# philbull/FastBox

Measured on AMD Instinct MI355X. Metric: 512^3 box realisations/sec (gen + log-normal + P(k)), higher is better.
Workload: dtype f32

## Files before the change

fastbox_amd/csrc/fb_api.hip:

```cpp
#include "../../include/fastbox_hip.h"
#include "fb_plan.h"
#include "fb_api_util.h"
#include <dlfcn.h>
#include <rccl/rccl.h>
#include <algorithm>
#include <cmath>
#include <cstdio>
#include <cstdlib>
#include <cstring>
#include <vector>

static thread_local std::string g_last_error;

void fb_set_error(const std::string& msg) { g_last_error = msg; }

int fb_hip_check(hipError_t e, const char* what) {
    if (e == hipSuccess) return FB_OK;
    g_last_error = std::string(what) + ": " + hipGetErrorString(e);
    (void)hipGetLastError();
    return e == hipErrorOutOfMemory ? FB_ERR_NOMEM : FB_ERR_HIP;
}

namespace {
template <typename T> int upload(T** dst, const T* src, size_t n) {
// ... 34 lines not shown
int fb_device_set(int device) {
    (void)hipGetLastError();
    FB_HIP(hipSetDevice(device));
    return FB_OK;
}

int fb_plan_create(fb_plan** plan, int N, double Lx, double Ly, double Lz, int precision, int device,
                   const double* axis2, const double* ksc, const double* kpar, const double* zgrid) {
    FB_REQUIRE(plan && axis2 && ksc && kpar && zgrid, "null pointer");
    FB_REQUIRE(precision == 4 || precision == 8, "precision must be 4 or 8");
    FB_REQUIRE(Lx > 0 && Ly > 0 && Lz > 0, "box sides must be positive");
    bool pow2 = N >= 16 && N <= 2048 && !(N & (N - 1)), smooth = false;
    if (!pow2 && N >= 16 && N <= 1024 && N % 2 == 0) {
        int q = N;
        for (int f : {2, 3, 5}) while (q % f == 0) q /= f;
        smooth = q == 1;
    }
    if (!pow2 && !smooth) {
        fb_set_error("unsupported grid size: nsamp must be a power of two in 16..2048, or even with prime factors 2, 3, 5 in 16..1024");
        return FB_ERR_UNSUPPORTED;
    }
    FB_HIP(hipSetDevice(device));
    fb_plan* p = new fb_plan();
    p->N = N; p->prec = precision; p->device = device;
    p->generic = pow2 ? 0 : 1;
    p->L[0] = Lx; p->L[1] = Ly; p->L[2] = Lz;
    p->cubic = (Lx == Ly && Ly == Lz);
    {
        hipDeviceProp_t prop;
        if (hipGetDeviceProperties(&prop, device) == hipSuccess && prop.multiProcessorCount > 0)
            p->num_cu = prop.multiProcessorCount;
    }
    p->NZV = N / 2 + 1;
    p->NZP = (p->NZV + 15) & ~15;
    p->NR = N + 1;
    int r = precision == 4 ? make_twiddles<float>(&p->tw, N) : make_twiddles<double>(&p->tw, N);
    if (!r) r = upload(&p->axis2, axis2, (size_t)3 * N);
    if (!r) r = upload(&p->ksc, ksc, (size_t)3 * N);
    if (!r) r = upload(&p->kpar, kpar, (size_t)N);
    if (!r) r = upload(&p->zgrid, zgrid, (size_t)N);
    if (!r) {
        std::vector<double> kp((size_t)N * N);
        for (int i = 0; i < N; ++i)
            for (int j = 0; j < N; ++j) kp[(size_t)i * N + j] = 6.283185307179586476925286766559 * std::sqrt(axis2[i] + axis2[N + j]);
        r = upload(&p->kperp_tab, kp.data(), kp.size());
    }
    p->prow = 2048;
    if (!r) r = fb_hip_check(hipMalloc((void**)&p->partials, (size_t)p->prow * 2 * FB_MAX_BINS * sizeof(double)), "hipMalloc");
    if (!r) r = fb_hip_check(hipMalloc((void**)&p->scratch, FB_SCRATCH * sizeof(double)), "hipMalloc");
    if (!r) r = fb_hip_check(hipMalloc((void**)&p->counts, FB_MAX_BINS * sizeof(unsigned long long)), "hipMalloc");
    if (!r) r = fb_hip_check(hipMalloc((void**)&p->bins, FB_MAX_BINS * sizeof(double)), "hipMalloc");
    if (!r) r = fb_hip_check(hipMalloc((void**)&p->thr, FB_MAX_BINS * sizeof(int)), "hipMalloc");
    if (!r) r = fb_hip_check(hipMalloc((void**)&p->plane_buf, (size_t)N * N * 2 * precision), "hipMalloc");
    if (r) { fb_plan_destroy(p); return r; }
    p->nbins = 0;
    *plan = p;
    return FB_OK;
}

int fb_comm_destroy(fb_plan* p);
int fb_plan_destroy(fb_plan* p) {
    if (!p) return FB_OK;
    (void)fb_comm_destroy(p);
    (void)hipSetDevice(p->device);
    void* ptrs[] = {p->tw, p->axis2, p->ksc, p->kpar, p->zgrid, p->amp_shell, p->amp_sym, p->kperp_tab, p->pca_work, p->bins, p->thr, p->counts,
                    p->partials, p->scratch, p->bin_partials, p->exp_partials, p->plane_buf, p->sep_edges, p->sep_partials,
                    p->halo_small, p->halo_work, p->halo_acc, p->pk_tab, p->pk_partials, p->void_small, p->void_work};
    for (void* q : ptrs) if (q) (void)hipFree(q);
    if (p->aux_stream) { (void)hipStreamSynchronize(p->aux_stream); (void)hipStreamDestroy(p->aux_stream); }
    if (p->ev_fork) (void)hipEventDestroy(p->ev_fork);
    if (p->ev_join) (void)hipEventDestroy(p->ev_join);
    for (hipEvent_t e : p->prof_ev) (void)hipEventDestroy(e);
    delete p;
    return FB_OK;
}

int fb_half_pitch(const fb_plan* p) { return p ? p->NZP : 0; }
int fb_half_rows(const fb_plan* p) { return p ? p->NR : 0; }
int64_t fb_real_bytes(const fb_plan* p) { return p ? (int64_t)p->N * p->N * p->N * p->prec : 0; }
int64_t fb_half_bytes(const fb_plan* p) { return p ? (int64_t)p->N * p->NR * p->NZP * 2 * p->prec : 0; }
int64_t fb_full_bytes(const fb_plan* p) { return p ? (int64_t)p->N * p->N * p->N * 2 * p->prec : 0; }

int fb_fft_c2c(fb_plan* p, void* d, int direction, double scale, void* stream) {
    FB_REQUIRE(p && d, "null pointer");
    FB_USE_DEVICE(p);
    FB_REQUIRE(direction == 1 || direction == -1, "direction must be +1 or -1");
    hipStream_t s = (hipStream_t)stream;
    return FB_DISPATCH(p, fbi_fft_c2c_f32(p, d, direction, scale, s), fbi_fft_c2c_f64(p, d, direction, scale, s));
}
int fb_fft_r2c(fb_plan* p, const void* in, void* out, int pre_exp, void* stream) {
    FB_REQUIRE(p && in && out, "null pointer");
    FB_USE_DEVICE(p);
    hipStream_t s = (hipStream_t)stream;
    return FB_DISPATCH(p, fbi_fft_r2c_f32(p, in, out, pre_exp, s), fbi_fft_r2c_f64(p, in, out, pre_exp, s));
}
int fb_fft_c2r(fb_plan* p, void* half, void* out, double scale, void* stream) {
    FB_REQUIRE(p && half && out, "null pointer");
    FB_USE_DEVICE(p);
    hipStream_t s = (hipStream_t)stream;
    return FB_DISPATCH(p, fbi_fft_c2r_f32(p, half, out, scale, s), fbi_fft_c2r_f64(p, half, out, scale, s));
}

#define FB_QUIESCE() FB_HIP(hipDeviceSynchronize())

int fb_set_amplitude_shells(fb_plan* p, const double* amp, int64_t nshell) {
    FB_REQUIRE(p && amp, "null pointer");
    FB_USE_DEVICE(p);
    FB_REQUIRE(p->cubic, "shell amplitudes need a cubic box (use fb_set_amplitude_dense)");
    const int64_t need = 3LL * (p->N / 2) * (p->N / 2) + 1;
    FB_REQUIRE(nshell == need, "nshell must be 3 (N/2)^2 + 1");
    FB_QUIESCE();
    p->amp_dense = nullptr;
    return FB_DISPATCH(p, fbi_set_amp_shells_f32(p, amp, nshell), fbi_set_amp_shells_f64(p, amp, nshell));
}
int fb_set_amplitude_sym(fb_plan* p, const double* amp, int64_t n) {
    FB_REQUIRE(p && amp, "null pointer");
    FB_USE_DEVICE(p);
    FB_QUIESCE();
    return FB_DISPATCH(p, fbi_set_amp_sym_f32(p, amp, n), fbi_set_amp_sym_f64(p, amp, n));
}
// ... 757 lines not shown
```

fastbox_amd/csrc/fb_fft_kernels.h:

```cpp
#pragma once
#include <type_traits>
#include "fb_fft.h"
#include "fb_field_kernels.h"

namespace fb {

#ifndef FB_E16_FROM
#define FB_E16_FROM 2048
#endif
constexpr int strided_elems(int n) { return n >= FB_E16_FROM ? 16 : fb_min(8, n); }

#ifndef FB_TILE_LINE
#define FB_TILE_LINE 128
#endif
template <typename T> constexpr int tile_cols(int n) {
    return fb_max(fb_max(2, fb_min(FB_TILE_LINE / (2 * (int)sizeof(T)),
                                   (n >= FB_E16_FROM ? (sizeof(T) == 8 ? 65536 : 131072) : 65536) / (n * 2 * (int)sizeof(T)))),
                  64 / (n / strided_elems(n)));
}

template <typename T> constexpr int strided_wg_per_cu(int n) {
    const int tile = n * tile_cols<T>(n) * 2 * (int)sizeof(T), nt = tile_cols<T>(n) * (n / strided_elems(n));
    return fb_max(1, fb_min(2048 / nt, tile > 81920 ? 1 : tile > 36864 ? 2 : 4));
}
// ... 21 lines not shown
#endif
#ifndef FB_ROW128_SWIZZLE
#define FB_ROW128_SWIZZLE 0
#endif
template <typename T> constexpr bool strided_row128(int n, int mode, bool blk) {
    return sizeof(T) == 4 && n == 2048 && !blk && mode != SMODE_BINF &&
           ((FB_ROW128_MODES >> (mode == SMODE_PLAIN ? 0 : (mode == SMODE_GEN ? 1 : 2))) & 1);
}
template <typename T> constexpr bool strided_split(int n, int mode, bool blk) {
    return strided_row128<T>(n, mode, blk) ||
           (sizeof(T) == 4 && n == 512 && !blk &&
            ((FB_SPLIT_MODES >> (mode == SMODE_PLAIN ? 0 : (mode == SMODE_GEN ? 1 : 2))) & 1));
}
#ifndef FB_GEN_WIDE_FROM
#define FB_GEN_WIDE_FROM 1024
#endif
template <typename T> constexpr bool strided_wide(int n, int mode, bool blk) {
    return sizeof(T) == 4 && mode == SMODE_GEN && !blk && n >= (FB_GEN_WIDE_FROM) && n >= 1024 && n < FB_E16_FROM;
}
template <typename T> constexpr int strided_elems_of(int n, int mode, bool blk) {
    return strided_row128<T>(n, mode, blk) ? 32 : ((strided_split<T>(n, mode, blk) || strided_wide<T>(n, mode, blk)) ? 16 : strided_elems(n));
}
template <typename T> constexpr int tile_cols_of(int n, int mode, bool blk) {
#ifndef FB_GEN_WIDE_COLS
#define FB_GEN_WIDE_COLS 16
#endif
    return strided_row128<T>(n, mode, blk) ? 16 : (strided_wide<T>(n, mode, blk) ? fb_min(FB_GEN_WIDE_COLS, 131072 / (n * 2 * (int)sizeof(T))) : tile_cols<T>(n));
}
template <typename T> constexpr int strided_wgs_of(int n, int mode, bool blk) {
    return strided_row128<T>(n, mode, blk) ? 1 : (strided_split<T>(n, mode, blk) ? FB_SPLIT_WGS : (strided_wide<T>(n, mode, blk) ? (FB_GEN_WIDE_COLS <= 8 ? 2 : 1) : strided_wg_per_cu<T>(n)));
}

template <typename T> struct StridedArgs {
    const cx<T>* in;
    cx<T>* out;
    const cx<T>* tw;
    long long stride;
    long long outer_stride;
    int ncols;
    T scale;
    int ntx;
    int ntiles;
    int drop_io;
    int wide;
    int ntx_shift;
    long long out_outer_stride;
    long long blk_stride;
    int blk_in, blk_out, blk_shift;
    int packed;
    int tile0;
    long long out_stride;
};

template <typename T> struct StridedOp {
    KGeom g;
    AmpSrc<T> amp;
    RngKey key;
    const int* thr;
    const double* bins;
    double* partial;
    long long partial_stride;
    cx<T>* plane_out;
    int nbins, namb, store;
    int outer0;
    int vel_on, vel_comp;
    double vel_fac;
    FilterSpec filt;
    const double* kperp_tab;
    int amb[8];
};

template <typename T, int N, int MODE, int PERSIST, bool BLK = false, int CSIGN = 0>
__global__ __launch_bounds__((tile_cols_of<T>(N, MODE, BLK) * (N / strided_elems_of<T>(N, MODE, BLK))),
                             fb_min(8, fb_max(1, strided_wgs_of<T>(N, MODE, BLK) * tile_cols_of<T>(N, MODE, BLK) * (N / strided_elems_of<T>(N, MODE, BLK)) / 256)))
void k_fft_strided(StridedArgs<T> a, int sign, StridedOp<T> op) {
    static_assert(!BLK || MODE == SMODE_PLAIN || MODE == SMODE_GEN || MODE == SMODE_BIN, "slab addressing: plain passes (and the generator / binning\n"
                  "pass of a k_z chunk, which keep the narrow tile the chunk bounds are counted in)");
    constexpr bool SPLIT = strided_split<T>(N, MODE, BLK);
    constexpr int E = strided_elems_of<T>(N, MODE, BLK);
    constexpr int TPL = N / E;
    constexpr int TZ = tile_cols_of<T>(N, MODE, BLK);
    constexpr int NT = TZ * TPL;
    constexpr int NW = (NT + 63) / 64;
    extern __shared__ __attribute__((aligned(16))) char smem[];
    cx<T>* twl = reinterpret_cast<cx<T>*>(smem + (size_t)N * TZ * (SPLIT ? sizeof(T) : sizeof(cx<T>)));
    double* acc = reinterpret_cast<double*>(twl + N);
    int* lthr = reinterpret_cast<int*>(acc + (size_t)NW * 2 * (smode_bins(MODE) ? op.nbins : 0));

    const int tid = threadIdx.x;
    const int c = tid % TZ;
    const int t = tid / TZ;
    auto load_tables = [&]() {
        for (int i = tid; i < N; i += NT) twl[i] = a.tw[i];
        if constexpr (smode_bins(MODE)) {
            for (int i = tid; i < NW * 2 * op.nbins; i += NT) acc[i] = 0.0;
            for (int i = tid; i < ((op.nbins + 63) & ~63); i += NT) lthr[i] = i < op.nbins ? op.thr[i] : 0x7fffffff;
        }
    };
    if constexpr (PERSIST) load_tables();
#ifdef FB_STAMPS
    long long* stamp = (smode_bins(MODE))
        ? reinterpret_cast<long long*>(op.partial + (size_t)2 * op.nbins * op.partial_stride) + (size_t)blockIdx.x * 32
        : reinterpret_cast<long long*>(const_cast<double*>(op.bins)) + (size_t)blockIdx.x * 32;
    const bool stamp_ok = (smode_bins(MODE)) ? (op.partial != nullptr) : (op.bins != nullptr);
#define FB_STAMP(k) do { if (tid == 0 && stamp_ok) stamp[k] = (long long)__builtin_amdgcn_s_memtime(); } while (0)
    FB_STAMP(0);
    if (tid == 0 && stamp_ok) {
        stamp[24] = (long long)__builtin_amdgcn_s_getreg((31 << 11) | 4);
        stamp[25] = (long long)__builtin_amdgcn_s_getreg((31 << 11) | 20);
    }
#else
#define FB_STAMP(k) do {} while (0)
#endif

    const int t0 = __builtin_amdgcn_readfirstlane(t);
    const long long tbase = (long long)t0 * a.stride;
    const unsigned loff = (unsigned)(((long long)(t - t0) * a.stride + c) * (long long)sizeof(cx<T>));
    const long long estep = (long long)TPL * a.stride;
    const unsigned estep_b = (unsigned)(estep * (long long)sizeof(cx<T>));
    [[maybe_unused]] auto eoff = [&](int e, int blocked, long long es) -> long long {
        return blocked ? (long long)(e >> a.blk_shift) * a.blk_stride + (long long)(e & ((1 << a.blk_shift) - 1)) * es
                       : (long long)e * es;
    };
// ... 3 lines not shown
    [[maybe_unused]] const long long estep_o = BLK ? (long long)TPL * ostride : estep;
    auto load_rows = [&](cx<T> (&r)[E], const cx<T>* src, const unsigned voff) {
        constexpr int AUX = smode_bins(MODE) ? FB_BIN_LOAD_AUX : 0;
        if constexpr (BLK) {
#pragma unroll
            for (int e = 0; e < E; ++e) r[e] = buf_load<AUX>(make_rsrc(src + eoff(e, a.blk_in, estep)), voff, 0u, src);
        } else if (!a.wide) {
            const __amdgpu_buffer_rsrc_t rs = make_rsrc(src);
#pragma unroll
            for (int e = 0; e < E; ++e) r[e] = buf_load<AUX>(rs, voff, (unsigned)e * estep_b, src);
        } else {
#pragma unroll
            for (int e = 0; e < E; ++e) r[e] = buf_load<AUX>(make_rsrc(src + (long long)e * estep), voff, 0u, src);
        }
    };
    auto store_rows = [&](cx<T>* dst, const unsigned voff, const cx<T> (&r)[E], const T scale) {
        constexpr int AUX = MODE == SMODE_GEN ? ((N == 1024 && !PERSIST && sizeof(T) == 4) ? 2 : FB_GEN_STORE_AUX) : 0;
        if constexpr (BLK) {
#pragma unroll
            for (int e = 0; e < E; ++e) buf_store<AUX>(make_rsrc(dst + eoff(e, a.blk_out, estep_o)), voff, 0u, cscale(r[e], scale));
        } else if (!a.wide) {
            const __amdgpu_buffer_rsrc_t rs = make_rsrc(dst);
#pragma unroll
            for (int e = 0; e < E; ++e) buf_store<AUX>(rs, voff, (unsigned)e * estep_b, cscale(r[e], scale));
        } else {
#pragma unroll
            for (int e = 0; e < E; ++e) buf_store<AUX>(make_rsrc(dst + (long long)e * estep), voff, 0u, cscale(r[e], scale));
        }
    };
    const long long out_outer = a.out_outer_stride ? a.out_outer_stride : a.outer_stride;

    cx<T> v[E];
    [[maybe_unused]] int wb_lo = 0, wb_hi = 0, wb_edge = 0x7fffffff;
    [[maybe_unused]] bool wb_ok = false, wb_rng = false;
    [[maybe_unused]] int thrv[4] = {0x7fffffff, 0x7fffffff, 0x7fffffff, 0x7fffffff};
    if constexpr (smode_bins(MODE) && !PERSIST) {
#pragma unroll
        for (int r = 0; r < 4; ++r)
            if (r * 64 < op.nbins) { const int q = r * 64 + (tid & 63); thrv[r] = q < op.nbins ? op.thr[q] : 0x7fffffff; }
    }
    [[maybe_unused]] auto wave_bin = [&](int n2) -> int {
        int b = 0;
#pragma unroll
        for (int r = 0; r < 4; ++r)
            if (r * 64 < op.nbins) {
                int th;
                if constexpr (PERSIST) th = lthr[r * 64 + (tid & 63)];
                else th = thrv[r];
                b += __builtin_popcountll(__ballot(th <= n2));
            }
        return b;
    };
    [[maybe_unused]] const int rot_rows = (int)gridDim.x >= a.ntx ? (int)gridDim.x / a.ntx : 1;
    auto place = [&](int id, int& bx, int& by) {
        const bool p2 = a.ntx_shift >= 0;
        bx = p2 ? (id & (a.ntx - 1)) : id % a.ntx;
        by = p2 ? (id >> a.ntx_shift) : id / a.ntx;
#ifndef FB_NO_TILE_ROTATE
        int rot = bx + by;
        if constexpr (PERSIST) rot += by / rot_rows;
        bx = p2 ? (rot & (a.ntx - 1)) : rot % a.ntx;
#endif
#ifndef FB_NO_XCD_PAIR
        if constexpr (TZ * sizeof(cx<T>) < 128) {
            constexpr int LPT = 128 / (TZ * (int)sizeof(cx<T>)), G = 8 * LPT;
            const int lg = bx % G;
            if (bx - lg + G <= a.ntx) bx = (bx - lg) + LPT * (lg % 8) + lg / 8;
        }
#endif
        bx += a.tile0;
    };
    int tile_id = blockIdx.x;
#ifndef FB_GEN_PARK
#define FB_GEN_PARK 16
#endif
    constexpr int PARK = (PERSIST && MODE == SMODE_GEN && !SPLIT && E == 16 && sizeof(T) == 4) ? FB_GEN_PARK : 0;
    constexpr int PARK0 = E - PARK;
    [[maybe_unused]] cx<T> wpark[PARK > 0 ? PARK : 1];
    [[maybe_unused]] bool staged = false;
    [[maybe_unused]] cx<T>* dst_prev = nullptr;
    [[maybe_unused]] unsigned voff_prev = FB_BUF_OOB;
    [[maybe_unused]] auto store_point = [&](cx<T>* dst, const unsigned voff, const int e, const cx<T> val) {
        if (!a.wide) buf_store<0>(make_rsrc(dst), voff, (unsigned)e * estep_b, val);
        else buf_store<0>(make_rsrc(dst + (long long)e * estep), voff, 0u, val);
    };
    [[maybe_unused]] auto drain = [&](auto slot_tag) {
        constexpr int S = decltype(slot_tag)::value;
        if constexpr (PARK > 0 && S >= 0 && S < 8) {
            constexpr int PER = PARK / 8;
            if (staged) {
                asm volatile("");
#pragma unroll
                for (int q = 0; q < PER; ++q) store_point(dst_prev, voff_prev, PARK0 + S * PER + q, wpark[S * PER + q]);
            }
        }
    };
#ifndef FB_BIN_DBUF
#define FB_BIN_DBUF 1
#endif
    constexpr bool DBUF = PERSIST && MODE == SMODE_BIN && !SPLIT && E == 16 && sizeof(T) == 4 && FB_BIN_DBUF;
    [[maybe_unused]] cx<T> vnext[DBUF ? E : 1];
    [[maybe_unused]] auto load_tile = [&](int id) {
        int lbx, lby;
        place(id, lbx, lby);
        const cx<T>* src = a.in + ((long long)lby * a.outer_stride + lbx * TZ + tbase);
        const unsigned voff = (id < a.ntiles && lbx * TZ + c < a.ncols && !a.drop_io) ? loff : FB_BUF_OOB;
        if constexpr (DBUF) load_rows(vnext, src, voff);
        else load_rows(v, src, voff);
    };
    if constexpr (MODE != SMODE_GEN && PERSIST) load_tile(tile_id);
    do {
        if constexpr (DBUF) {
#pragma unroll
            for (int e = 0; e < E; ++e) v[e] = vnext[e];
            load_tile(tile_id + (int)gridDim.x);
        }
        int tid_tile = tid;
        if constexpr (PERSIST) asm volatile("" : "+v"(tid_tile));
        const int tid = tid_tile, c = tid % TZ, t = tid / TZ;
        int bx, by;
        place(tile_id, bx, by);
        const int col = bx * TZ + c;
        const bool valid = col < a.ncols;
        const long long ubase = (long long)by * a.outer_stride + bx * TZ;
// ... 390 lines not shown
#pragma unroll 1
                for (int q = 0; q < E; ++q) {
                    const int kz = col0 + (off0 + q) % TZ;
                    const int n2 = mode_n2(q);
                    const double w = (n2 < 0) ? 0.0 : ((kz == 0 || kz == (N >> 1)) ? 1.0 : 2.0);
                    const double p = (double)ptile[off0 + q];
                    const bool up = n2 >= edge;
                    s1 += up ? 0.0 : w * p; s2 += up ? 0.0 : w * p * p;
                    u1 += up ? w * p : 0.0; u2 += up ? w * p * p : 0.0;
                }
                wave_flush(blo, s1, s2, any_ok && blo < nb, row);
                if (__any(any_ok && bhi > blo)) wave_flush(bhi, u1, u2, any_ok && bhi > blo && bhi < nb, row);
            } else {
#pragma unroll 1
                for (int q = 0; q < E; ++q) {
                    const int kx = (off0 + q) / TZ, kz = col0 + (off0 + q) % TZ;
                    const int n2 = mode_n2(q);
                    int bb = n2 >= 0 ? shell_bin(lthr, nb, n2) : nb;
                    for (int z = 0; z < op.namb; ++z)
                        if (n2 >= 0 && op.amb[z] == n2) bb = bin_exact(op.bins, nb, kmag_exact(op.g, kx, ky, kz));
                    const double w = (kz == 0 || kz == (N >> 1)) ? 1.0 : 2.0;
                    const double p = (double)ptile[off0 + q];
                    wave_flush(bb, w * p, w * p * p, n2 >= 0 && bb < nb, row);
                }
            }
            }
        }
#ifdef FB_STAMPS
        if constexpr (!smode_bins(MODE)) FB_STAMP(5);
        asm volatile("s_waitcnt vmcnt(0)" ::: "memory");
        FB_STAMP(6);
#endif
        if constexpr (!PERSIST) break;
        tile_id += gridDim.x;
    } while (tile_id < a.ntiles);
    if constexpr (PARK > 0) {
        if (staged) {
#pragma unroll
            for (int e = 0; e < PARK; ++e) store_point(dst_prev, voff_prev, PARK0 + e, wpark[e]);
        }
    }
    if constexpr (smode_bins(MODE)) {
#ifdef FB_STAMPS
        if ((tid & 63) == 0 && stamp_ok) stamp[8 + (tid >> 6)] = (long long)__builtin_amdgcn_s_memtime();
#endif
        __syncthreads();
        const int nb = op.nbins;
        for (int i = tid; i < 2 * nb; i += NT) {
            double sum = 0.0;
            for (int w2 = 0; w2 < NW; ++w2) sum += acc[(size_t)w2 * 2 * nb + i];
            op.partial[(size_t)i * op.partial_stride + blockIdx.x] = sum;
        }
        FB_STAMP(7);
    }
}

static __global__ __launch_bounds__(1024) void k_sum_columns(const double* __restrict__ partial, long long nrows,
                                                              int nvals, double* __restrict__ out,
                                                              const double* __restrict__ partial2, long long nrows2,
                                                              long long stride = 0) {
    __shared__ double sh[1024];
    const int q = blockIdx.x, nt = blockDim.x;
    const double* src = partial + (size_t)q * (stride ? stride : nrows);
    if (q == nvals) {
        if (!partial2) { if (threadIdx.x == 0) out[q] = 0.0; return; }
        src = partial2; nrows = nrows2;
    }
    double c[8] = {0, 0, 0, 0, 0, 0, 0, 0};
    long long r = threadIdx.x;
    for (; r + 7 * nt < nrows; r += 8 * nt) {
#pragma unroll
        for (int u = 0; u < 8; ++u) c[u] += src[r + u * nt];
    }
    for (int u = 0; r < nrows; r += nt, ++u) c[u & 7] += src[r];
    const double s = ((c[0] + c[1]) + (c[2] + c[3])) + ((c[4] + c[5]) + (c[6] + c[7]));
    sh[threadIdx.x] = s;
    __syncthreads();
    for (int o = nt >> 1; o > 0; o >>= 1) {
        if ((int)threadIdx.x < o) sh[threadIdx.x] += sh[threadIdx.x + o];
        __syncthreads();
    }
    if (threadIdx.x == 0) out[q] = sh[0];
}

template <typename T>
__global__ __launch_bounds__(256) void k_bin_packed_plane(const cx<T>* __restrict__ plane, KGeom g, BinGeom bg,
                                                           double* __restrict__ partial, long long stride, long long col0) {
    extern __shared__ __attribute__((aligned(16))) char smem[];
    double* lbins = reinterpret_cast<double*>(smem);
    double* acc = lbins + bg.nbins;
    int* lthr = reinterpret_cast<int*>(acc + 4 * 2 * bg.nbins);
    const int N = g.N, nb = bg.nbins, tid = threadIdx.x;
    for (int q = tid; q < nb; q += 256) { lbins[q] = bg.bins[q]; lthr[q] = bg.thr ? bg.thr[q] : 0; }
    for (int q = tid; q < 8 * nb; q += 256) acc[q] = 0.0;
    __syncthreads();
    const int ky = blockIdx.x, kym = (N - ky) & (N - 1);
    double* row = acc + (size_t)(tid >> 6) * 2 * nb;
    for (int kx0 = 0; kx0 < N; kx0 += 256) {
        const int kx = kx0 + tid;
        const bool have = kx < N;
        cx<T> G{0, 0}, M{0, 0};
        if (have) { G = plane[(long long)ky * N + kx]; M = plane[(long long)kym * N + ((N - kx) & (N - 1))]; }
        const cx<T> x0{(T)0.5 * (G.x + M.x), (T)0.5 * (G.y - M.y)};
        const cx<T> x1{(T)0.5 * (G.y + M.y), (T)0.5 * (M.x - G.x)};
        const T p0 = x0.x * x0.x + x0.y * x0.y, p1 = x1.x * x1.x + x1.y * x1.y;
        const int b0 = have ? bin_of_mode(bg, g, lbins, lthr, kx, ky, 0) : nb;
        const int b1 = have ? bin_of_mode(bg, g, lbins, lthr, kx, ky, N >> 1) : nb;
        wave_flush(b0, p0, p0 * p0, have && b0 < nb, row);
        wave_flush(b1, p1, p1 * p1, have && b1 < nb, row);
    }
    __syncthreads();
    for (int i = tid; i < 2 * nb; i += 256)
        partial[(size_t)i * stride + col0 + blockIdx.x] = (acc[i] + acc[2 * nb + i]) + (acc[4 * nb + i] + acc[6 * nb + i]);
}

__device__ __forceinline__ double fb_exp(double x) { return exp(x); }
__device__ __forceinline__ float fb_exp(float x) {
#ifdef FB_LIBM_EXP
    return expf(x);
#else
    const float t = x * 1.44269502162933349609375f;
    float e = __builtin_fmaf(x, 1.44269502162933349609375f, -t);
    e = __builtin_fmaf(x, 1.925963033500011e-8f, e);
    const float r = __builtin_amdgcn_exp2f(t);
    return r > 3.4028234663852886e38f ? r : __builtin_fmaf(r, 0.693147182464599609375f * e, r);
#endif
}
enum { ZMODE_C2C = 0, ZMODE_R2C = 1, ZMODE_C2R = 2, ZMODE_C2R2C = 3 };

template <typename T> struct ContigArgs {
    const void* in;
    void* out;
    const cx<T>* tw;
    long long in_pitch;
    long long out_pitch;
    int in_skip, out_skip;
    long long nlines;
    T scale;
    int pre_exp;
    double* exp_partial;
    void* out2;
    int packed;
    T exp_shift;
};

#ifndef FB_CONTIG_THREADS
#define FB_CONTIG_THREADS 256
#endif
template <typename T, int NF> constexpr int contig_lines() {
    return fb_max(1, FB_CONTIG_THREADS / (NF / elems_per_thread<T>(NF)));
}

template <typename T, int NF, bool WAVE>
__device__ __forceinline__ void c2r_line(const cx<T>* __restrict__ in, const int packed, const int t, const cx<T>* twl,
                                         const LineLayout<T>& lay, const T scale, cx<T> (&v)[elems_per_thread<T>(NF)]) {
    constexpr int E = elems_per_thread<T>(NF), TPL = NF / E;
#pragma unroll
    for (int e = 0; e < E; ++e) {
// ... 282 lines not shown
```

fastbox_amd/csrc/fb_fft_launch.inc:

```
#include <cstdlib>
#include <cstring>
#include "fb_plan.h"
#include "fb_fft_kernels.h"
#include "fb_fft_generic.h"

namespace {

using namespace fb;
typedef FB_REAL real_t;
typedef cx<real_t> cplx_t;

template <typename K> int set_lds(K kernel, size_t bytes) {
    if (bytes > 65536)
        FB_HIP(hipFuncSetAttribute(reinterpret_cast<const void*>(kernel),
                                   hipFuncAttributeMaxDynamicSharedMemorySize, (int)bytes));
    return FB_OK;
}

KGeom fft_geom(const fb_plan* p) { return KGeom{p->axis2, p->ksc, p->kpar, p->N, p->NZV, p->NZP, p->NR}; }
int gen_amplitude(const fb_plan* p, StridedOp<real_t>& op) {
    op.amp.shell = (p->amp_dense || p->amp_sym_only) ? nullptr : reinterpret_cast<const real_t*>(p->amp_shell);
    op.amp.dense = p->amp_sym_only ? nullptr : reinterpret_cast<const real_t*>(p->amp_dense);
    op.amp.sym = (op.amp.shell || p->amp_sym_only) ? reinterpret_cast<const real_t*>(p->amp_sym) : nullptr;
    if (!op.amp.shell && !op.amp.dense && !op.amp.sym) { fb_set_error("amplitude table not set (fb_set_amplitude_*)"); return FB_ERR_STATE; }
    return FB_OK;
}

int ensure(double** buf, size_t* cap, size_t need) {
    if (*cap >= need) return FB_OK;
    if (*buf) FB_HIP(hipFree(*buf));
    *buf = nullptr; *cap = 0;
    FB_HIP(hipMalloc(reinterpret_cast<void**>(buf), need * sizeof(double)));
    *cap = need;
    return FB_OK;
}

template <int N, int MODE, int PERSIST, bool BLK>
int launch_strided_npb(fb_plan* p, const StridedArgs<real_t>& a, int nouter, int sign, StridedOp<real_t>& op,
                       hipStream_t s) {
    constexpr bool SPLIT = strided_split<real_t>(N, MODE, BLK);
    constexpr int E = strided_elems_of<real_t>(N, MODE, BLK), TPL = N / E, TZ = tile_cols_of<real_t>(N, MODE, BLK);
    constexpr int NW = (TZ * TPL + 63) / 64;
    size_t lds = (size_t)N * TZ * (SPLIT ? sizeof(real_t) : sizeof(cplx_t)) + (size_t)N * sizeof(cplx_t);
    if (smode_bins(MODE)) lds += (size_t)NW * 2 * op.nbins * sizeof(double) + (size_t)((op.nbins + 63) & ~63) * sizeof(int);
    StridedArgs<real_t> b = a;
    b.ntx = a.ntx ? a.ntx : (a.ncols + TZ - 1) / TZ;
    b.ntiles = b.ntx * nouter;
    b.ntx_shift = -1;
    for (int q = 0; q < 30; ++q) if ((1 << q) == b.ntx) b.ntx_shift = q;
    b.wide = ((long long)(E - 1) * TPL * a.stride * (long long)sizeof(cplx_t) >= 0xE0000000LL) ? 1 : 0;
    b.drop_io = p->debug_no_mem;
    auto pick = [&]() {
#ifndef FB_CSIGN_FROM
#define FB_CSIGN_FROM (1 << 30)
#endif
        if constexpr (MODE == SMODE_PLAIN && (strided_row128<real_t>(N, MODE, BLK) || N >= (FB_CSIGN_FROM)))
            return sign < 0 ? k_fft_strided<real_t, N, MODE, PERSIST, BLK, -1> : k_fft_strided<real_t, N, MODE, PERSIST, BLK, +1>;
        else return k_fft_strided<real_t, N, MODE, PERSIST, BLK>;
    };
    auto kernel = pick();
    int r = set_lds(kernel, lds);
    if (r) return r;
    int nblk = b.ntiles;
    if (PERSIST) {
        static thread_local int per_cu = 0;
        static thread_local size_t per_cu_lds = 0;
        if (!per_cu || per_cu_lds != lds) {
            int q = 1;
            FB_HIP(hipOccupancyMaxActiveBlocksPerMultiprocessor(&q, kernel, TZ * TPL, lds));
            per_cu = q < 1 ? 1 : (q > 4 ? 4 : q);
            per_cu_lds = lds;
        }
        if (per_cu * p->num_cu < nblk) nblk = per_cu * p->num_cu;
    }
    if (smode_bins(MODE) && p->bin_append_cap && !a.ntx) p->bin_append_cap = 0;
    if (smode_bins(MODE) && p->bin_append_cap) {
        if (p->bin_rows + nblk > p->bin_append_cap) { fb_set_error("binning chunks exceed the partial-sum table"); return FB_ERR_STATE; }
        op.partial = p->bin_partials + p->bin_rows;
        op.partial_stride = p->bin_append_cap;
        p->bin_rows += nblk;
        p->bin_rows_main = p->bin_rows;
    } else if (smode_bins(MODE)) {
        const long long rows = nblk + (a.packed ? N : 0);
#ifdef FB_STAMPS
        r = ensure(&p->bin_partials, &p->bin_partials_cap, (size_t)rows * 2 * op.nbins + (size_t)nblk * 32 + 64);
#else
        r = ensure(&p->bin_partials, &p->bin_partials_cap, (size_t)rows * 2 * op.nbins);
#endif
        if (r) return r;
        op.partial = p->bin_partials;
        op.partial_stride = rows;
        p->bin_rows = rows;
        p->bin_rows_main = nblk;
    }
    { FbProfScope _ps(p, MODE == SMODE_GEN ? FBK_FFT_GEN : (smode_bins(MODE) ? FBK_FFT_BIN : FBK_FFT_STRIDED), s);
    hipLaunchKernelGGL(kernel, dim3(nblk), dim3(TZ * TPL), lds, s, b, sign, op); }
    FB_LAUNCH_CHECK("k_fft_strided");
    return FB_OK;
}
#ifndef FB_WIDE_ROWS_DEFAULT
#define FB_WIDE_ROWS_DEFAULT 1
#endif
template <int N, int MODE, int PERSIST>
int launch_strided_np(fb_plan* p, const StridedArgs<real_t>& a, int nouter, int sign, StridedOp<real_t>& op,
                      hipStream_t s) {
    if constexpr (MODE == SMODE_PLAIN) {
        if (a.blk_in || a.blk_out) return launch_strided_npb<N, MODE, PERSIST, true>(p, a, nouter, sign, op, s);
    }
    if constexpr (MODE == SMODE_GEN && strided_wide<real_t>(N, MODE, false)) {
        if (a.ntx || a.tile0) return launch_strided_npb<N, MODE, PERSIST, true>(p, a, nouter, sign, op, s);
    }
    if constexpr (strided_row128<real_t>(N, MODE, false)) {
        static const char* env = getenv("FB_WIDE_ROWS");
        const int mask = env ? atoi(env) : (p->wide_rows >= 0 ? p->wide_rows : FB_WIDE_ROWS_DEFAULT);
        const int bit = MODE == SMODE_PLAIN ? 1 : (MODE == SMODE_GEN ? 2 : 4);
        if (!(mask & bit) || a.ntx || a.tile0) return launch_strided_npb<N, MODE, PERSIST, true>(p, a, nouter, sign, op, s);
    }
    return launch_strided_npb<N, MODE, PERSIST, false>(p, a, nouter, sign, op, s);
}

template <int N, int MODE>
int launch_strided_n(fb_plan* p, const StridedArgs<real_t>& a, int nouter, int sign, StridedOp<real_t>& op,
                     hipStream_t s) {
    if constexpr (N >= 256 && MODE != SMODE_BINF) {
        static const char* env = getenv("FB_PASS_SCHEDULE");
        const int cls = MODE == SMODE_GEN ? 1 : (smode_bins(MODE) ? 2 : 0);
        static const bool env_ok = env && strlen(env) == 3 && strspn(env, "01") == 3;
        int sched = env_ok ? env[cls] - '0' : p->pass_schedule[cls];
        if (sched < 0) sched = strided_elems_of<real_t>(N, MODE, MODE == SMODE_GEN && (a.ntx || a.tile0)) > 8 ? 1 : 0;
        if (sched == 1) return launch_strided_np<N, MODE, 1>(p, a, nouter, sign, op, s);
    }
    return launch_strided_np<N, MODE, 0>(p, a, nouter, sign, op, s);
}

template <int MODE>
int launch_strided(fb_plan* p, int N, const StridedArgs<real_t>& a, int nouter, int sign, StridedOp<real_t>& op,
                   hipStream_t s) {
    switch (N) {
        case 16: return launch_strided_n<16, MODE>(p, a, nouter, sign, op, s);
        case 32: return launch_strided_n<32, MODE>(p, a, nouter, sign, op, s);
        case 64: return launch_strided_n<64, MODE>(p, a, nouter, sign, op, s);
        case 128: return launch_strided_n<128, MODE>(p, a, nouter, sign, op, s);
        case 256: return launch_strided_n<256, MODE>(p, a, nouter, sign, op, s);
        case 512: return launch_strided_n<512, MODE>(p, a, nouter, sign, op, s);
        case 1024: return launch_strided_n<1024, MODE>(p, a, nouter, sign, op, s);
        case 2048: return launch_strided_n<2048, MODE>(p, a, nouter, sign, op, s);
    }
// ... 153 lines not shown
int join_streams(fb_plan* p, const PlaneBatches& pb, hipStream_t s) {
    if (pb.streams < 2) return FB_OK;
    FB_HIP(hipEventRecord(p->ev_join, p->aux_stream));
    FB_HIP(hipStreamWaitEvent(s, p->ev_join, 0));
    return FB_OK;
}

template <int ZM>
int yz_passes(fb_plan* p, cplx_t* h, const void* real_in, void* real_out, bool y_before, bool y_after, double scale,
              int pre_exp, hipStream_t s, bool packed = false) {
    const int N = p->N;
    const long long hplane = (long long)p->NR * p->NZP, rplane = (long long)N * N;
    const PlaneBatches pb = plane_batches(p, (size_t)hplane * sizeof(cplx_t) + (size_t)rplane * sizeof(real_t));
    int r = FB_OK;
    if (pre_exp && pb.count > 1) {
        r = ensure(&p->exp_partials, &p->exp_partials_cap, (size_t)rplane + (size_t)pb.count);
        if (r) return r;
    }
    r = fork_streams(p, pb, s);
    if (r) return r;
    p->exp_base = 0;
    for (int b = 0; b < pb.count && !r; ++b) {
        const int p0 = b * pb.per, cnt = (p0 + pb.per <= N) ? pb.per : N - p0;
        hipStream_t st = (pb.streams > 1 && (b & 1)) ? p->aux_stream : s;
        cplx_t* hb = h + p0 * hplane;
        if (y_before) r = launch_plain(p, N, half_y(p, hb, packed), cnt, +1, st);
        if (r) break;
        if (ZM == ZMODE_R2C) {
            ContigArgs<real_t> az{reinterpret_cast<const real_t*>(real_in) + p0 * rplane, hb, (const cplx_t*)p->tw, (long long)N,
                                  (long long)p->NZP, 0, N, cnt * (long long)N, (real_t)1, pre_exp, nullptr, nullptr, packed};
            r = launch_contig<ZM>(p, N / 2, az, -1, st);
        } else {
            ContigArgs<real_t> az{hb, real_out ? reinterpret_cast<real_t*>(real_out) + p0 * rplane : nullptr, (const cplx_t*)p->tw, (long long)p->NZP,
                                  (long long)N, N, 0, cnt * (long long)N, (real_t)scale, pre_exp, nullptr,
                                  ZM == ZMODE_C2R2C ? hb : nullptr, packed};
            r = launch_contig<ZM>(p, N / 2, az, +1, st);
        }
        if (r) break;
        p->exp_base = p->exp_rows;
        if (y_after) r = launch_plain(p, N, half_y(p, hb, packed), cnt, -1, st);
    }
    p->exp_base = 0;
    const int rj = join_streams(p, pb, s);
    return r ? r : rj;
}

int bin_x_pass(fb_plan* p, cplx_t* h, bool packed, int pre_exp, double* results, hipStream_t s) {
    const int N = p->N, nb = p->nbins;
    StridedOp<real_t> op = {};
    op.g = fft_geom(p);
    op.thr = p->thr; op.bins = p->bins; op.nbins = nb; op.namb = p->namb; op.store = 0;
    for (int q = 0; q < 8; ++q) op.amb[q] = p->amb[q];
    op.plane_out = packed ? reinterpret_cast<cplx_t*>(p->plane_buf) : nullptr;
    int r = launch_strided<SMODE_BIN>(p, N, half_x(p, h, packed), N, -1, op, s);
    if (r) return r;
    if (packed) {
        BinGeom bg;
        bg.bins = p->bins; bg.thr = p->use_thr ? p->thr : nullptr; bg.nbins = nb; bg.namb = p->namb;
        for (int q = 0; q < 8; ++q) bg.amb[q] = p->amb[q];
        const size_t lds = (size_t)nb * sizeof(double) + (size_t)8 * nb * sizeof(double) + (size_t)nb * sizeof(int);
        { FbProfScope _ps(p, FBK_BIN, s);
        hipLaunchKernelGGL(k_bin_packed_plane<real_t>, dim3(N), dim3(256), lds, s, reinterpret_cast<const cplx_t*>(p->plane_buf),
                           op.g, bg, p->bin_partials, p->bin_rows, p->bin_rows_main); }
        FB_LAUNCH_CHECK("k_bin_packed_plane");
    }
    { FbProfScope _ps(p, FBK_BIN, s);
    hipLaunchKernelGGL(k_sum_columns, dim3(2 * nb + 1), dim3(1024), 0, s, p->bin_partials, p->bin_rows, 2 * nb, results,
                       pre_exp ? p->exp_partials : nullptr, (long long)p->exp_rows, 0LL); }
    FB_LAUNCH_CHECK("k_sum_columns");
    return FB_OK;
}

int filtered_x_pass(fb_plan* p, cplx_t* h, int kind, const double* prm, const void* table, double* results, int inverse_x,
                    hipStream_t s) {
    const int N = p->N, nb = p->nbins;
    StridedOp<real_t> op = {};
    op.g = fft_geom(p);
    op.thr = p->thr; op.bins = p->bins; op.nbins = nb; op.namb = p->namb; op.store = inverse_x ? 2 : 1;
    for (int q = 0; q < 8; ++q) op.amb[q] = p->amb[q];
    op.filt.kind = kind; op.filt.table = table;
    for (int q = 0; q < 4; ++q) op.filt.p[q] = prm ? prm[q] : 0.0;
    op.kperp_tab = p->kperp_tab;
    int r = launch_strided<SMODE_BINF>(p, N, half_x(p, h), N, -1, op, s);
    if (r) return r;
    { FbProfScope _ps(p, FBK_BIN, s);
    hipLaunchKernelGGL(k_sum_columns, dim3(2 * nb + 1), dim3(1024), 0, s, p->bin_partials, p->bin_rows, 2 * nb, results,
                       (const double*)nullptr, 0LL, 0LL); }
    FB_LAUNCH_CHECK("k_sum_columns");
    return FB_OK;
}
int filter_args_ok(const fb_plan* p, int kind, const void* table) {
    if (!p->nbins || !p->use_thr) { fb_set_error("fused P(k) needs shell thresholds (fb_set_bins with thr)"); return FB_ERR_STATE; }
    if (kind < 0 || kind > FILT_TOPHAT) { fb_set_error("unknown filter kind"); return FB_ERR_INVALID; }
    if (kind == FILT_TOPHAT) {
        fb_set_error("the fused filtering pass takes FB_FILT_TABLE, _BEAM_HIGHPASS and _WEDGE; apply FB_FILT_TOPHAT with fb_apply_filter");
        return FB_ERR_UNSUPPORTED;
    }
    if (kind == FILT_TABLE && !table) { fb_set_error("FB_FILT_TABLE needs a device table"); return FB_ERR_INVALID; }
    return FB_OK;
}

template <int E_>
int launch_rsd_turn(fb_plan* p, const RsdTurnArgs<real_t>& a, hipStream_t s) {
    if constexpr (sizeof(real_t) == 4) {
        constexpr size_t lds = rsd_turn_lds<E_>();
        int r = set_lds(k_rsd_turn<real_t, E_>, lds);
        if (r) return r;
        const unsigned nb = (unsigned)((a.nlines + FB_RSDT_WAVES - 1) / FB_RSDT_WAVES);
// ... 618 lines not shown
```

fastbox_amd/csrc/fb_plan.h:

```cpp
#pragma once
#include <hip/hip_runtime.h>
#include <stdint.h>
#include <string>
#include <vector>

#define FB_OK 0
#define FB_ERR_INVALID -1
#define FB_ERR_HIP -2
#define FB_ERR_UNSUPPORTED -3
#define FB_ERR_NOMEM -4
#define FB_ERR_STATE -5
#define FB_ERR_RCCL -6

struct fb_comm;

struct fb_plan {
    fb_comm* comm = nullptr;
    int N = 0;
    int generic = 0;
    int prec = 4;
    double L[3] = {0, 0, 0};
    int device = 0;
    int debug_no_mem = 0;
    int pass_schedule[3] = {-1, -1, -1};
    int wide_rows = -1;
    int plane_batch = -1;
    int plane_streams = 0;
    double exp_shift = 0.0;
    int num_cu = 256;
    int NZV = 0;
    int NZP = 0;
    int NR = 0;
    int cubic = 0;

    void* tw = nullptr;
    double* axis2 = nullptr;
    double* kpar = nullptr;
    double* ksc = nullptr;
    double* zgrid = nullptr;

    void* amp_shell = nullptr;
    int64_t nshell = 0;
    const void* amp_dense = nullptr;
    void* pca_work = nullptr;
    size_t pca_work_cap = 0;
    double* kperp_tab = nullptr;
    int amp_sym_only = 0;
    void* amp_sym = nullptr;

    double* bins = nullptr;
    int nbins = 0;
    int* thr = nullptr;
    int use_thr = 0;
    int namb = 0;
    int amb[8] = {0, 0, 0, 0, 0, 0, 0, 0};
    unsigned long long* counts = nullptr;
    double counts_host[256];
    double* partials = nullptr;
    int prow = 0;
    double* scratch = nullptr;
    double* bin_partials = nullptr;
    size_t bin_partials_cap = 0;
    long long bin_rows = 0;
    long long bin_rows_main = 0;
    long long bin_append_cap = 0;
    void* plane_buf = nullptr;
    double* exp_partials = nullptr;
    size_t exp_partials_cap = 0;
    long long exp_rows = 0;
    long long exp_base = 0;

    double* sep_edges = nullptr;
    std::vector<std::vector<double>> sep_geom;
    double* sep_partials = nullptr;
    size_t sep_partials_cap = 0;

    double* pk_tab = nullptr;
    double* pk_partials = nullptr;
    size_t pk_partials_cap = 0;
    std::vector<std::vector<double>> pk_geom;

    void* halo_small = nullptr;
    void* halo_work = nullptr;
    size_t halo_work_cap = 0;
    void* halo_acc = nullptr;
    size_t halo_acc_cap = 0;

    void* void_small = nullptr;
    void* void_work = nullptr;
    size_t void_work_cap = 0;

    hipStream_t aux_stream = nullptr;
    hipEvent_t ev_fork = nullptr, ev_join = nullptr;

    bool prof_on = false;
    unsigned prof_mask = 0xFFFFFFFFu;
    int prof_stride = 1;
    long long prof_seen = 0;
    std::vector<hipEvent_t> prof_ev;
    std::vector<int> prof_cat;
    size_t prof_used = 0;
};

enum { FBK_FFT_STRIDED = 0, FBK_FFT_CONTIG, FBK_COLOUR, FBK_BIN, FBK_FILTER, FBK_VELPOT, FBK_REALOP, FBK_RSD,
       FBK_LAYOUT, FBK_FFT_GEN, FBK_FFT_BIN, FBK_PCA, FBK_NCAT };

struct FbProfScope {
    fb_plan* p; hipStream_t s; size_t slot; bool on;
    FbProfScope(fb_plan* plan, int cat, hipStream_t stream)
        : p(plan), s(stream), slot(0), on(plan->prof_on && ((plan->prof_mask >> cat) & 1u)) {
        if (!on) return;
        if ((p->prof_seen++ % p->prof_stride) != 0) { on = false; return; }
        if (p->prof_used + 2 > p->prof_ev.size()) {
            for (int q = 0; q < 64; ++q) { hipEvent_t e; if (hipEventCreate(&e) != hipSuccess) { on = false; return; }
                                           p->prof_ev.push_back(e); }
        }
        slot = p->prof_used; p->prof_used += 2;
        p->prof_cat.resize(p->prof_used / 2); p->prof_cat[slot / 2] = cat;
        (void)hipEventRecord(p->prof_ev[slot], s);
// ... 110 lines not shown
```

Baseline: 1069.

## Fold packed-plane binning and column reduction into binning FFT kernel tail

Adds a last-block-done ticket scheme so the strided binning FFT kernel itself bins the packed k_z=0/Nyquist planes and reduces the per-block partials hierarchically into final results. This removes two separate kernel launches (k_bin_packed_plane and k_sum_columns) and their launch gaps from the P(k) path. It introduces atomic tickets, release/acquire fences and extra LDS, and it is enabled by default via FB_BIN_TAIL. The added tail work is serialised onto whichever blocks finish last.

```diff
diff --git a/fastbox_amd/csrc/fb_api.hip b/fastbox_amd/csrc/fb_api.hip
--- a/fastbox_amd/csrc/fb_api.hip
+++ b/fastbox_amd/csrc/fb_api.hip
@@ -110,6 +110,12 @@
     if (!r) r = fb_hip_check(hipMalloc((void**)&p->bins, FB_MAX_BINS * sizeof(double)), "hipMalloc");
     if (!r) r = fb_hip_check(hipMalloc((void**)&p->thr, FB_MAX_BINS * sizeof(int)), "hipMalloc");
     if (!r) r = fb_hip_check(hipMalloc((void**)&p->plane_buf, (size_t)N * N * 2 * precision), "hipMalloc");
+    if (const char* env = getenv("FB_BIN_TAIL")) p->bin_tail = atoi(env) != 0;
+    if (!r && pow2) {
+        const size_t nt = (size_t)N / 2 + 1 + 128 + 1;
+        r = fb_hip_check(hipMalloc((void**)&p->tail_tickets, nt * sizeof(int)), "hipMalloc");
+        if (!r) r = fb_hip_check(hipMemset(p->tail_tickets, 0, nt * sizeof(int)), "hipMemset");
+    }
     if (r) { fb_plan_destroy(p); return r; }
     p->nbins = 0;
     *plan = p;
@@ -123,7 +129,7 @@
     (void)hipSetDevice(p->device);
     void* ptrs[] = {p->tw, p->axis2, p->ksc, p->kpar, p->zgrid, p->amp_shell, p->amp_sym, p->kperp_tab, p->pca_work, p->bins, p->thr, p->counts,
                     p->partials, p->scratch, p->bin_partials, p->exp_partials, p->plane_buf, p->sep_edges, p->sep_partials,
-                    p->halo_small, p->halo_work, p->halo_acc, p->pk_tab, p->pk_partials, p->void_small, p->void_work};
+                    p->halo_small, p->halo_work, p->halo_acc, p->pk_tab, p->pk_partials, p->void_small, p->void_work, p->tail_tickets};
     for (void* q : ptrs) if (q) (void)hipFree(q);
     if (p->aux_stream) { (void)hipStreamSynchronize(p->aux_stream); (void)hipStreamDestroy(p->aux_stream); }
     if (p->ev_fork) (void)hipEventDestroy(p->ev_fork);
diff --git a/fastbox_amd/csrc/fb_fft_kernels.h b/fastbox_amd/csrc/fb_fft_kernels.h
--- a/fastbox_amd/csrc/fb_fft_kernels.h
+++ b/fastbox_amd/csrc/fb_fft_kernels.h
@@ -97,6 +97,18 @@
     long long out_stride;
 };
 
+struct BinTail {
+    int* tickets;
+    double* grows;
+    double* results;
+    const double* exp_partial;
+    long long exp_rows;
+    long long col0;
+    int ng, gsize;
+    int npg, psize;
+    unsigned lds_off;
+};
+
 template <typename T> struct StridedOp {
     KGeom g;
     AmpSrc<T> amp;
@@ -106,6 +118,7 @@
     double* partial;
     long long partial_stride;
     cx<T>* plane_out;
+    BinTail tail;
     int nbins, namb, store;
     int outer0;
     int vel_on, vel_comp;
@@ -114,6 +127,162 @@
     const double* kperp_tab;
     int amb[8];
 };
+
+template <typename T>
+__device__ __forceinline__ void plane_powers(const cx<T> G, const cx<T> M, T& p0, T& p1) {
+    const cx<T> x0{(T)0.5 * (G.x + M.x), (T)0.5 * (G.y - M.y)};
+    const cx<T> x1{(T)0.5 * (G.y + M.y), (T)0.5 * (M.x - G.x)};
+    if constexpr (sizeof(T) == 4) {
+        p0 = __builtin_fmaf(x0.y, x0.y, x0.x * x0.x);
+        p1 = __builtin_fmaf(x1.x, x1.x, x1.y * x1.y);
+    } else {
+        p0 = __builtin_fma(x0.y, x0.y, x0.x * x0.x);
+        p1 = __builtin_fma(x1.x, x1.x, x1.y * x1.y);
+    }
+}
+
+__device__ __forceinline__ bool tail_ticket(int* ticket, int expect, int* flag) {
+    asm volatile("s_waitcnt vmcnt(0)" ::: "memory");
+    __syncthreads();
+    if (threadIdx.x == 0) {
+        __builtin_amdgcn_fence(__ATOMIC_RELEASE, "agent");
+        asm volatile("s_waitcnt vmcnt(0)" ::: "memory");
+        const int old = __hip_atomic_fetch_add(ticket, 1, __ATOMIC_RELAXED, __HIP_MEMORY_SCOPE_AGENT);
+        const int last = old == expect - 1 ? 1 : 0;
+        if (last) {
+            __builtin_amdgcn_fence(__ATOMIC_ACQUIRE, "agent");
+            asm volatile("s_waitcnt vmcnt(0)" ::: "memory");
+        }
+        *flag = last;
+    }
+    __syncthreads();
+    return __builtin_amdgcn_readfirstlane(*flag) != 0;
+}
+template <typename RowOf>
+__device__ __forceinline__ void tail_sum_rows(const double* src, long long stride, int nvals, int nrows, RowOf row_of,
+                                              const double* src2, long long nrows2, double* out, long long ostride) {
+    const int lane = threadIdx.x & 63, wid = threadIdx.x >> 6, nw = ((int)blockDim.x + 63) >> 6;
+    for (int i = wid; i < nvals + (src2 ? 1 : 0); i += nw) {
+        double s = 0.0;
+        if (i < nvals) {
+            const double* col = src + (size_t)i * stride;
+#pragma unroll 4
+            for (int j = lane; j < nrows; j += 64) { const long long r = row_of(j); s += r >= 0 ? col[r] : 0.0; }
+        } else {
+#pragma unroll 4
+            for (long long j = lane; j < nrows2; j += 64) s += src2[j];
+        }
+        s = wave_sum(s);
+        if (lane == 0) out[(size_t)i * ostride] = s;
+    }
+}
+template <typename T> struct StridedKArgs { StridedArgs<T> a; int sign; StridedOp<T> op; };
+template <typename T, typename KP, typename PlaceIn>
+__device__ __forceinline__ void bin_tail(KP kp, const size_t lthr_off0, const int nw_rows, PlaceIn place_in) {
+    extern __shared__ __attribute__((aligned(16))) char smem[];
+    auto fresh = [&]() -> const StridedKArgs<T>* { KP q = kp; asm volatile("" : "+s"(q)); return (const StridedKArgs<T>*)q; };
+    const int tid = threadIdx.x, nt = blockDim.x;
+    auto scratch = [&](const StridedOp<T>& op) -> char* { return smem + op.tail.lds_off; };
+    auto group_done = [&]() {
+        const StridedOp<T>& op = fresh()->op;
+        const BinTail& tl = op.tail;
+        const int nb = op.nbins, npairs = (op.g.N >> 1) + 1, ngr = tl.ng + tl.npg;
+        if (!tail_ticket(tl.tickets + npairs + ngr, ngr, reinterpret_cast<int*>(scratch(op)))) return;
+        tail_sum_rows(tl.grows, (long long)ngr, 2 * nb, ngr, [](int j) -> long long { return j; },
+                      (const double*)nullptr, 0LL, tl.results, 1LL);
+        if (tl.exp_partial)
+            tail_sum_rows(tl.grows + (size_t)2 * nb * ngr, (long long)ngr, 1, tl.ng, [](int j) -> long long { return j; },
+                          (const double*)nullptr, 0LL, tl.results + 2 * nb, 1LL);
+        else if (tid == 0) tl.results[2 * nb] = 0.0;
+        for (int q = tid; q < npairs + ngr + 1; q += nt) tl.tickets[q] = 0;
+    };
+    auto bin_plane_row = [&](int ky) {
+        const StridedOp<T>& op = fresh()->op;
+        const int N = op.g.N, nb = op.nbins;
+        double* lbins = reinterpret_cast<double*>(scratch(op) + 8);
+        double* pacc = lbins + nb;
+        const int* lthr = reinterpret_cast<const int*>(smem + lthr_off0 + (size_t)nw_rows * 2 * nb * sizeof(double));
+        auto bin_of = [&](int i, int j, int l) -> int {
+            const int n2 = shell_of(i, j, l, N);
+            bool amb = false;
+            for (int q = 0; q < op.namb; ++q) amb |= (op.amb[q] == n2);
+            return amb ? bin_exact(lbins, nb, kmag_exact(op.g, i, j, l)) : shell_bin(lthr, nb, n2);
+        };
+        const cx<T>* plane = op.plane_out;
+        const int kym = (N - ky) & (N - 1);
+        for (int q = tid; q < nb; q += nt) lbins[q] = op.bins[q];
+        for (int q = tid; q < 8 * nb; q += nt) pacc[q] = 0.0;
+        __syncthreads();
+        for (int vw = tid >> 6; vw < 4; vw += (nt + 63) >> 6) {
+            double* row = pacc + (size_t)vw * 2 * nb;
+            for (int kx0 = 0; kx0 < N; kx0 += 256) {
+                const int kx = kx0 + vw * 64 + (tid & 63);
+                const bool have = kx < N;
+                cx<T> G{0, 0}, M{0, 0};
+                if (have) { G = plane[(long long)ky * N + kx]; M = plane[(long long)kym * N + ((N - kx) & (N - 1))]; }
+                T p0, p1;
+                plane_powers(G, M, p0, p1);
+                const int b0 = have ? bin_of(kx, ky, 0) : nb;
+                const int b1 = have ? bin_of(kx, ky, N >> 1) : nb;
+                wave_flush(b0, p0, p0 * p0, have && b0 < nb, row);
+                wave_flush(b1, p1, p1 * p1, have && b1 < nb, row);
+            }
+        }
+        __syncthreads();
+        for (int i = tid; i < 2 * nb; i += nt)
+            op.partial[(size_t)i * op.partial_stride + op.tail.col0 + ky] = (pacc[i] + pacc[2 * nb + i]) + (pacc[4 * nb + i] + pacc[6 * nb + i]);
+        __syncthreads();
+    };
+    auto plane_group = [&](int pr) {
+        const StridedOp<T>& op = fresh()->op;
+        const BinTail& tl = op.tail;
+        const int N = op.g.N, npairs = (N >> 1) + 1, ngr = tl.ng + tl.npg;
+        const int pg = pr / tl.psize, p0 = pg * tl.psize;
+        const int p1 = p0 + tl.psize < npairs ? p0 + tl.psize : npairs;
+        if (!tail_ticket(tl.tickets + npairs + pg, p1 - p0, reinterpret_cast<int*>(scratch(op)))) return;
+        const long long c0 = tl.col0;
+        tail_sum_rows(op.partial, op.partial_stride, 2 * op.nbins, 2 * (p1 - p0),
+                      [=](int j) -> long long {
+                          const int pp = p0 + (j >> 1);
+                          if (!(j & 1)) return c0 + pp;
+                          return (pp == 0 || 2 * pp == N) ? -1LL : c0 + (N - pp);
+                      },
+                      (const double*)nullptr, 0LL, tl.grows + tl.ng + pg, (long long)ngr);
+        group_done();
+    };
+    if (fresh()->op.tail.npg) {
+        for (int id = blockIdx.x; id < fresh()->a.ntiles; id += gridDim.x) {
+            int bx, by;
+            {
+                const StridedArgs<T>& a = fresh()->a;
+                place_in(a, (int)gridDim.x >= a.ntx ? (int)gridDim.x / a.ntx : 1, id, bx, by);
+            }
+            if (bx != 0) continue;
+            const StridedOp<T>& op = fresh()->op;
+            const int N = op.g.N;
+            const int ky = by + op.outer0, kym = (N - ky) & (N - 1);
+            const int pr = ky < kym ? ky : kym;
+            if (!tail_ticket(op.tail.tickets + pr, ky == kym ? 1 : 2, reinterpret_cast<int*>(scratch(op)))) continue;
+            bin_plane_row(ky);
+            if (kym != ky) bin_plane_row(kym);
+            plane_group(pr);
+        }
+    }
+    {
+        const StridedOp<T>& op = fresh()->op;
+        const BinTail& tl = op.tail;
+        const int npairs = (op.g.N >> 1) + 1, ngr = tl.ng + tl.npg;
+        const int g = (int)blockIdx.x / tl.gsize, r0 = g * tl.gsize;
+        const int r1 = r0 + tl.gsize < (int)gridDim.x ? r0 + tl.gsize : (int)gridDim.x;
+        if (!tail_ticket(tl.tickets + npairs + tl.npg + g, r1 - r0, reinterpret_cast<int*>(scratch(op)))) return;
+        const long long es = (tl.exp_rows + tl.ng - 1) / tl.ng, e0 = g * es;
+        const long long e1 = e0 + es < tl.exp_rows ? e0 + es : tl.exp_rows;
+        tail_sum_rows(op.partial, op.partial_stride, 2 * op.nbins, r1 - r0, [=](int j) -> long long { return r0 + j; },
+                      tl.exp_partial ? tl.exp_partial + (e0 < e1 ? e0 : 0) : nullptr, e1 > e0 ? e1 - e0 : 0LL,
+                      tl.grows + g, (long long)ngr);
+    }
+    group_done();
+}
 
 template <typename T, int N, int MODE, int PERSIST, bool BLK = false, int CSIGN = 0>
 __global__ __launch_bounds__((tile_cols_of<T>(N, MODE, BLK) * (N / strided_elems_of<T>(N, MODE, BLK))),
@@ -223,7 +392,7 @@
         return b;
     };
     [[maybe_unused]] const int rot_rows = (int)gridDim.x >= a.ntx ? (int)gridDim.x / a.ntx : 1;
-    auto place = [&](int id, int& bx, int& by) {
+    auto place_in = [](const StridedArgs<T>& a, const int rot_rows, int id, int& bx, int& by) {
         const bool p2 = a.ntx_shift >= 0;
         bx = p2 ? (id & (a.ntx - 1)) : id % a.ntx;
         by = p2 ? (id >> a.ntx_shift) : id / a.ntx;
@@ -241,6 +410,7 @@
 #endif
         bx += a.tile0;
     };
+    auto place = [&](int id, int& bx, int& by) { place_in(a, rot_rows, id, bx, by); };
     int tile_id = blockIdx.x;
 #ifndef FB_GEN_PARK
 #define FB_GEN_PARK 16
@@ -737,6 +907,15 @@
             op.partial[(size_t)i * op.partial_stride + blockIdx.x] = sum;
         }
         FB_STAMP(7);
+        if constexpr (MODE == SMODE_BIN) {
+            auto kp = __builtin_amdgcn_kernarg_segment_ptr();
+            asm volatile("" : "+s"(kp));
+            if (((const StridedKArgs<T>*)kp)->op.tail.tickets) {
+                asm volatile("");
+                constexpr size_t FRONT = (size_t)N * TZ * (SPLIT ? sizeof(T) : sizeof(cx<T>)) + (size_t)N * sizeof(cx<T>);
+                bin_tail<T>(kp, FRONT, NW, place_in);
+            }
+        }
     }
 }
 
@@ -786,9 +965,8 @@
         const bool have = kx < N;
         cx<T> G{0, 0}, M{0, 0};
         if (have) { G = plane[(long long)ky * N + kx]; M = plane[(long long)kym * N + ((N - kx) & (N - 1))]; }
-        const cx<T> x0{(T)0.5 * (G.x + M.x), (T)0.5 * (G.y - M.y)};
-        const cx<T> x1{(T)0.5 * (G.y + M.y), (T)0.5 * (M.x - G.x)};
-        const T p0 = x0.x * x0.x + x0.y * x0.y, p1 = x1.x * x1.x + x1.y * x1.y;
+        T p0, p1;
+        plane_powers(G, M, p0, p1);
         const int b0 = have ? bin_of_mode(bg, g, lbins, lthr, kx, ky, 0) : nb;
         const int b1 = have ? bin_of_mode(bg, g, lbins, lthr, kx, ky, N >> 1) : nb;
         wave_flush(b0, p0, p0 * p0, have && b0 < nb, row);
diff --git a/fastbox_amd/csrc/fb_fft_launch.inc b/fastbox_amd/csrc/fb_fft_launch.inc
--- a/fastbox_amd/csrc/fb_fft_launch.inc
+++ b/fastbox_amd/csrc/fb_fft_launch.inc
@@ -43,6 +43,12 @@
     constexpr int NW = (TZ * TPL + 63) / 64;
     size_t lds = (size_t)N * TZ * (SPLIT ? sizeof(real_t) : sizeof(cplx_t)) + (size_t)N * sizeof(cplx_t);
     if (smode_bins(MODE)) lds += (size_t)NW * 2 * op.nbins * sizeof(double) + (size_t)((op.nbins + 63) & ~63) * sizeof(int);
+    if (smode_bins(MODE) && op.tail.tickets) {
+        const size_t front = (size_t)N * TZ * (SPLIT ? sizeof(real_t) : sizeof(cplx_t)) + (size_t)N * sizeof(cplx_t);
+        const size_t need = 8 + (size_t)72 * op.nbins;
+        op.tail.lds_off = need <= front ? 0u : (unsigned)lds;
+        if (need > front) lds += need;
+    }
     StridedArgs<real_t> b = a;
     b.ntx = a.ntx ? a.ntx : (a.ncols + TZ - 1) / TZ;
     b.ntiles = b.ntx * nouter;
@@ -85,14 +91,25 @@
 #ifdef FB_STAMPS
         r = ensure(&p->bin_partials, &p->bin_partials_cap, (size_t)rows * 2 * op.nbins + (size_t)nblk * 32 + 64);
 #else
-        r = ensure(&p->bin_partials, &p->bin_partials_cap, (size_t)rows * 2 * op.nbins);
+        r = ensure(&p->bin_partials, &p->bin_partials_cap, (size_t)rows * 2 * op.nbins + (size_t)128 * (2 * op.nbins + 1));
 #endif
         if (r) return r;
         op.partial = p->bin_partials;
         op.partial_stride = rows;
         p->bin_rows = rows;
         p->bin_rows_main = nblk;
-    }
+        if (op.tail.tickets) {
+            BinTail& tl = op.tail;
+            const int npairs = N / 2 + 1;
+            tl.gsize = (nblk + 63) / 64;
+            tl.ng = (nblk + tl.gsize - 1) / tl.gsize;
+            tl.psize = (npairs + 63) / 64;
+            tl.npg = a.packed ? (npairs + tl.psize - 1) / tl.psize : 0;
+            tl.col0 = nblk;
+            tl.grows = p->bin_partials + (size_t)rows * 2 * op.nbins;
+        }
+    }
+    if (smode_bins(MODE) && p->bin_append_cap) op.tail.tickets = nullptr;
     { FbProfScope _ps(p, MODE == SMODE_GEN ? FBK_FFT_GEN : (smode_bins(MODE) ? FBK_FFT_BIN : FBK_FFT_STRIDED), s);
     hipLaunchKernelGGL(kernel, dim3(nblk), dim3(TZ * TPL), lds, s, b, sign, op); }
     FB_LAUNCH_CHECK("k_fft_strided");
@@ -352,8 +369,13 @@
     op.thr = p->thr; op.bins = p->bins; op.nbins = nb; op.namb = p->namb; op.store = 0;
     for (int q = 0; q < 8; ++q) op.amb[q] = p->amb[q];
     op.plane_out = packed ? reinterpret_cast<cplx_t*>(p->plane_buf) : nullptr;
+    const bool fold = p->bin_tail && p->tail_tickets && p->use_thr;
+    if (fold) {
+        op.tail.tickets = p->tail_tickets; op.tail.results = results;
+        op.tail.exp_partial = pre_exp ? p->exp_partials : nullptr; op.tail.exp_rows = p->exp_rows;
+    }
     int r = launch_strided<SMODE_BIN>(p, N, half_x(p, h, packed), N, -1, op, s);
-    if (r) return r;
+    if (r || fold) return r;
     if (packed) {
         BinGeom bg;
         bg.bins = p->bins; bg.thr = p->use_thr ? p->thr : nullptr; bg.nbins = nb; bg.namb = p->namb;
diff --git a/fastbox_amd/csrc/fb_plan.h b/fastbox_amd/csrc/fb_plan.h
--- a/fastbox_amd/csrc/fb_plan.h
+++ b/fastbox_amd/csrc/fb_plan.h
@@ -65,6 +65,8 @@
     long long bin_rows_main = 0;
     long long bin_append_cap = 0;
     void* plane_buf = nullptr;
+    int bin_tail = 1;
+    int* tail_tickets = nullptr;
     double* exp_partials = nullptr;
     size_t exp_partials_cap = 0;
     long long exp_rows = 0;
```

Measured after the change: 738.9. -30.9%, worse.
